# jianzhnie/ScaleRL

Hardware: NVIDIA H100
Metric: learner_frames_per_sec (higher is better)
Workload: dtype bf16

## Files before the change

### scalerl_b200/csrc/igemm_tma.cuh

```cuda
#pragma once
#include <cuda.h>
#include "common.cuh"
#include "kernels.h"

namespace srl {

SRL_DEVINL void tma_prefetch_desc(const CUtensorMap* m) {
  asm volatile("prefetch.tensormap [%0];" ::"l"(reinterpret_cast<uint64_t>(m)) : "memory");
}
SRL_DEVINL void tma_load_2d(void* dst, const CUtensorMap* m, uint64_t* bar, int c0, int c1) {
  asm volatile("cp.async.bulk.tensor.2d.shared::cluster.global.mbarrier::complete_tx::bytes [%0], [%1, {%3, %4}], [%2];"
               ::"r"(smem_u32(dst)), "l"(reinterpret_cast<uint64_t>(m)), "r"(smem_u32(bar)), "r"(c0), "r"(c1) : "memory");
}
SRL_DEVINL void tma_load_3d(void* dst, const CUtensorMap* m, uint64_t* bar, int c0, int c1, int c2) {
  asm volatile("cp.async.bulk.tensor.3d.shared::cluster.global.mbarrier::complete_tx::bytes [%0], [%1, {%3, %4, %5}], [%2];"
               ::"r"(smem_u32(dst)), "l"(reinterpret_cast<uint64_t>(m)), "r"(smem_u32(bar)), "r"(c0), "r"(c1), "r"(c2) : "memory");
}
SRL_DEVINL void tma_load_4d(void* dst, const CUtensorMap* m, uint64_t* bar, int c0, int c1, int c2, int c3) {
  asm volatile("cp.async.bulk.tensor.4d.shared::cluster.global.mbarrier::complete_tx::bytes [%0], [%1, {%3, %4, %5, %6}], [%2];"
               ::"r"(smem_u32(dst)), "l"(reinterpret_cast<uint64_t>(m)), "r"(smem_u32(bar)), "r"(c0), "r"(c1), "r"(c2), "r"(c3)
               : "memory");
}
SRL_DEVINL void tma_load_5d(void* dst, const CUtensorMap* m, uint64_t* bar, int c0, int c1, int c2, int c3, int c4) {
  asm volatile("cp.async.bulk.tensor.5d.shared::cluster.global.mbarrier::complete_tx::bytes [%0], [%1, {%3, %4, %5, %6, %7}], [%2];"
               ::"r"(smem_u32(dst)), "l"(reinterpret_cast<uint64_t>(m)), "r"(smem_u32(bar)), "r"(c0), "r"(c1), "r"(c2), "r"(c3), "r"(c4)
               : "memory");
}

constexpr int IGT_THREADS = 288;

template <class P, int SPLIT = 0>
struct TmaCfg {
  static constexpr int KROWS = P::A_MN ? P::KROWS : 64;
  static constexpr int A_BYTES = P::A_MN ? 2 * KROWS * 128 : 128 * 128;
  static constexpr int B_BLOCKS = (P::BN + 63) / 64;
  static constexpr int B_BYTES = P::B_MN ? B_BLOCKS * KROWS * 128 : P::BN * 128;
  static constexpr int HALF_BYTES = A_BYTES + B_BYTES;
  static constexpr int STAGE_BYTES = HALF_BYTES * (1 + SPLIT);
  static constexpr int NB = P::BN / 2;
  static constexpr int STAGES = fit_stages(P::STAGES, 2 * WG_IMG_BYTES + 1024 + 256, STAGE_BYTES);
  static constexpr int SMEM_BYTES = STAGES * STAGE_BYTES + 2 * WG_IMG_BYTES + 1024 + 256;
  static_assert(SMEM_BYTES <= 232448, "shared memory budget (227 KB)");
  static_assert(NB == 32 || NB == 64 || NB == 128, "MMA N per warpgroup");
  static constexpr int MMAS = P::A_MN ? KROWS / 16 : 4;
  static_assert(A_BYTES % 1024 == 0 && B_BYTES % 1024 == 0, "operand tiles must keep 1024 B alignment (SWIZZLE_128B atoms)");
  static_assert(P::A_MN == P::B_MN, "mixed majors are not used");
  static_assert(KROWS % 16 == 0, "contraction rows per stage must be a multiple of MMA K = 16");
};

template <class P, int SPLIT>
SRL_DEVINL void igt_epilogue(const typename P::Params& p, int tm, int ty, int row, int c0, float (&v)[16]) {
  if constexpr (SPLIT) P::template epilogue16<1>(p, tm, ty, row, c0, v); else P::epilogue16(p, tm, ty, row, c0, v);
}
template <class P, int SPLIT>
SRL_DEVINL void igt_epilogue(const typename P::Params& p, int tm, int ty, int row, int c0, float (&v)[16], const uint4 (&pre)[2]) {
  if constexpr (SPLIT) P::template epilogue16<1>(p, tm, ty, row, c0, v, pre); else P::epilogue16(p, tm, ty, row, c0, v, pre);
}

template <class P, int SPLIT = 0>
__global__ void __launch_bounds__(IGT_THREADS) igemm_tma_kernel(const __grid_constant__ typename P::Params p) {
  using C = TmaCfg<P, SPLIT>;
  extern __shared__ uint8_t smem_raw[];
  uint8_t* smem = reinterpret_cast<uint8_t*>((reinterpret_cast<uintptr_t>(smem_raw) + 1023) & ~uintptr_t(1023));
  float* img = reinterpret_cast<float*>(smem + C::STAGES * C::STAGE_BYTES);
  uint64_t* bars = reinterpret_cast<uint64_t*>(smem + C::STAGES * C::STAGE_BYTES + 2 * WG_IMG_BYTES);
  uint64_t* full = bars;
  uint64_t* empty = bars + C::STAGES;

  const int tid = threadIdx.x;
  const int warp = tid >> 5;
  const int tm = blockIdx.x, ty = blockIdx.y;
  const int nkb = P::num_kblocks(p, tm, ty);

  if constexpr (P::ZERO_INIT) {
    if (P::zero_cta(ty)) {
      uint4* z = reinterpret_cast<uint4*>(smem);
      for (int i = tid; i < C::STAGES * C::STAGE_BYTES / 16; i += IGT_THREADS) z[i] = make_uint4(0, 0, 0, 0);
    }
    __syncthreads();
    for (int s = 0; s < C::STAGES; ++s) P::init_smem(p, tm, ty, smem + s * C::STAGE_BYTES, tid);
    fence_proxy_async_smem();
  }
  if (warp == 8 && (tid & 31) == 0) {
    for (int s = 0; s < C::STAGES; ++s) { mbar_init(&full[s], 1); mbar_init(&empty[s], 8); }
    mbar_fence_init();
    P::prefetch(p);
  }
  __syncthreads();
  pdl_wait(P::KID);
  if (tid == 256) pdl_launch();

  if (warp == 8) {
    const uint32_t leader = elect_one_sync();
    for (int kb = 0; kb < nkb; ++kb) {
      const int s = kb % C::STAGES;
      mbar_wait(&empty[s], ((kb / C::STAGES) & 1) ^ 1);
      if (leader) {
        uint8_t* sA = smem + s * C::STAGE_BYTES;
        if constexpr (SPLIT) P::issue_split(p, tm, ty, kb, sA, C::A_BYTES, C::HALF_BYTES, &full[s]);
        else P::issue(p, tm, ty, kb, sA, sA + C::A_BYTES, &full[s]);
      }
      __syncwarp();
    }
  } else {
    const int g = warp >> 2, wt = tid & 127;
    constexpr int NB = C::NB;
    uint4 pre[P::PREFETCH ? NB / 16 : 1][2];
    if constexpr (P::PREFETCH) {
#pragma unroll
      for (int c = 0; c < NB / 16; ++c) P::prefetch16(p, tm, ty, wt, g * NB + c * 16, pre[c]);
    }
    float acc[2][NB / 2];
#pragma unroll
    for (int h = 0; h < 2; ++h)
#pragma unroll
      for (int i = 0; i < NB / 2; ++i) acc[h][i] = 0.f;
    constexpr uint32_t ASTEP = P::A_MN ? 2048 / 16 : 32 / 16, BSTEP = P::B_MN ? 2048 / 16 : 32 / 16;
    constexpr uint32_t A_HI = (P::A_MN ? C::KROWS * 128 : 64 * 128) / 16;
    const uint32_t b_off = P::B_MN ? (g * NB / 64) * C::KROWS * 128 + (g * NB % 64) * 2 : g * NB * 128;
    for (int kb = 0; kb < nkb; ++kb) {
      const int s = kb % C::STAGES;
      mbar_wait(&full[s], (kb / C::STAGES) & 1);
      const uint32_t a0 = smem_u32(smem + s * C::STAGE_BYTES);
      const uint64_t ad0 = P::A_MN ? make_smem_desc(a0, C::KROWS * 128, 1024) : make_smem_desc(a0, 16, 1024);
      const uint64_t bd0 = P::B_MN ? make_smem_desc(a0 + C::A_BYTES + b_off, C::KROWS * 128, 1024) : make_smem_desc(a0 + C::A_BYTES + b_off, 16, 1024);
      wg_fence();
#pragma unroll
      for (int k = 0; k < C::MMAS; ++k) {
        const uint64_t ad = ad0 + (uint64_t)(k * ASTEP), bd = bd0 + (uint64_t)(k * BSTEP);
        wg_mma128<NB, P::A_MN ? 1 : 0, P::B_MN ? 1 : 0>(acc, ad, A_HI, bd, (kb | k) != 0);
        if constexpr (SPLIT) {
          wg_mma128<NB, P::A_MN ? 1 : 0, P::B_MN ? 1 : 0>(acc, ad, A_HI, bd + (uint64_t)(C::HALF_BYTES / 16), 1);
          wg_mma128<NB, P::A_MN ? 1 : 0, P::B_MN ? 1 : 0>(acc, ad + (uint64_t)(C::HALF_BYTES / 16), A_HI, bd, 1);
        }
      }
      wg_commit();
      if constexpr (C::STAGES > 1) {
        wg_wait_prev();
        __syncwarp();
        if (kb > 0 && (tid & 31) == 0) mbar_arrive(&empty[(kb - 1) % C::STAGES]);
      } else {
        wg_wait_all();
        __syncwarp();
        if ((tid & 31) == 0) mbar_arrive(&empty[s]);
      }
    }
    wg_wait_all();
    wg_fence_regs(acc[0]); wg_fence_regs(acc[1]);
    float* my_img = img + g * (WG_IMG_BYTES / 4);
#pragma unroll
    for (int c = 0; c < NB / 16; ++c) {
      float v[16];
      wg_acc_row16<NB>(acc, c, my_img, wt, 2 + g, v);
      if constexpr (P::PREFETCH) igt_epilogue<P, SPLIT>(p, tm, ty, wt, g * NB + c * 16, v, pre[c]);
      else igt_epilogue<P, SPLIT>(p, tm, ty, wt, g * NB + c * 16, v);
    }
  }
}

template <class P, int SPLIT = 0>
cudaError_t igemm_tma_launch(const typename P::Params& p, dim3 grid, cudaStream_t stream) {
  using C = TmaCfg<P, SPLIT>;
  if (grid.x == 0 || grid.y == 0) return cudaSuccess;
  static PerDeviceOnce once;
  { cudaError_t e = ensure_max_dynamic_smem(once, igemm_tma_kernel<P, SPLIT>, C::SMEM_BYTES); if (e != cudaSuccess) return e; }
  return launch_chain(igemm_tma_kernel<P, SPLIT>, grid, dim3(IGT_THREADS), C::SMEM_BYTES, stream, p);
}

}
```

### scalerl_b200/csrc/tma_problems.cuh

```cuda
#pragma once
#include "igemm_tma.cuh"
#include "encoder_problems.cuh"

namespace srl {

#define SRL_TMAP alignas(64) CUtensorMap

struct TFcFwd {
  static constexpr int KID = 31;
  static constexpr bool PREFETCH = false;
  static constexpr int BN = 64, STAGES = 4, SPLITS = 4;
  static constexpr bool A_MN = false, B_MN = false, ZERO_INIT = false;
  static constexpr int KROWS = 64;
  struct Params { SRL_TMAP a3m; SRL_TMAP w; SRL_TMAP a3m_lo; SRL_TMAP w_lo; float* out; int M; };
  SRL_DEVINL static void prefetch(const Params& p) { tma_prefetch_desc(&p.a3m); tma_prefetch_desc(&p.w); }
  SRL_DEVINL static int kb_begin(int split) { return (49 * split) / SPLITS; }
  SRL_DEVINL static void issue_split(const Params& p, int tm, int ty, int kb, uint8_t* st, int a_bytes, int half, uint64_t* bar) {
    const int k = (kb_begin(ty % SPLITS) + kb) * 64;
    mbar_arrive_expect_tx(bar, 2 * (128 * 128 + 64 * 128));
    tma_load_2d(st, &p.a3m, bar, k, tm * 128);
    tma_load_2d(st + a_bytes, &p.w, bar, k, (ty / SPLITS) * 64);
    tma_load_2d(st + half, &p.a3m_lo, bar, k, tm * 128);
    tma_load_2d(st + half + a_bytes, &p.w_lo, bar, k, (ty / SPLITS) * 64);
  }
  template <int SPLIT>
  SRL_DEVINL static void epilogue16(const Params& p, int tm, int ty, int row, int c0, float (&v)[16]) { epilogue16(p, tm, ty, row, c0, v); }
  SRL_DEVINL static int num_kblocks(const Params&, int, int ty) { const int sp = ty % SPLITS; return kb_begin(sp + 1) - kb_begin(sp); }
  SRL_DEVINL static void issue(const Params& p, int tm, int ty, int kb, uint8_t* sA, uint8_t* sB, uint64_t* bar) {
    const int k = (kb_begin(ty % SPLITS) + kb) * 64;
    mbar_arrive_expect_tx(bar, 128 * 128 + 64 * 128);
    tma_load_2d(sA, &p.a3m, bar, k, tm * 128);
    tma_load_2d(sB, &p.w, bar, k, (ty / SPLITS) * 64);
  }
  SRL_DEVINL static void epilogue16(const Params& p, int tm, int ty, int row, int c0, float (&v)[16]) {
    const int m = tm * 128 + row;
    if (m >= p.M) return;
    float4* o = reinterpret_cast<float4*>(p.out + ((size_t)(ty % SPLITS) * p.M + m) * 512 + (ty / SPLITS) * 64 + c0);
#pragma unroll
    for (int j = 0; j < 4; ++j) o[j] = make_float4(v[4 * j], v[4 * j + 1], v[4 * j + 2], v[4 * j + 3]);
  }
};

struct TFcDgrad {
  static constexpr int KID = 32;
  static constexpr bool PREFETCH = true;
  static constexpr int BN = 64, STAGES = 4;
  static constexpr bool A_MN = false, B_MN = false, ZERO_INIT = false;
  static constexpr int KROWS = 64;
  struct Params { SRL_TMAP dhm; SRL_TMAP w; SRL_TMAP dhm_lo; SRL_TMAP w_lo; const bf16* a3; bf16* da3; bf16* da3_lo; int M; };
  SRL_DEVINL static void prefetch(const Params& p) { tma_prefetch_desc(&p.dhm); tma_prefetch_desc(&p.w); }
  SRL_DEVINL static int num_kblocks(const Params&, int, int) { return 8; }
  SRL_DEVINL static void issue_split(const Params& p, int tm, int ty, int kb, uint8_t* st, int a_bytes, int half, uint64_t* bar) {
    mbar_arrive_expect_tx(bar, 2 * (128 * 128 + 64 * 128));
    tma_load_2d(st, &p.dhm, bar, kb * 64, tm * 128);
    tma_load_2d(st + a_bytes, &p.w, bar, kb * 64, ty * 64);
    tma_load_2d(st + half, &p.dhm_lo, bar, kb * 64, tm * 128);
    tma_load_2d(st + half + a_bytes, &p.w_lo, bar, kb * 64, ty * 64);
  }
  SRL_DEVINL static void issue(const Params& p, int tm, int ty, int kb, uint8_t* sA, uint8_t* sB, uint64_t* bar) {
    mbar_arrive_expect_tx(bar, 128 * 128 + 64 * 128);
    tma_load_2d(sA, &p.dhm, bar, kb * 64, tm * 128);
    tma_load_2d(sB, &p.w, bar, kb * 64, ty * 64);
  }
  SRL_DEVINL static void prefetch16(const Params& p, int tm, int ty, int row, int c0, uint4 (&mk)[2]) {
    const int m = tm * 128 + row;
    if (m < p.M) ld_mask16(p.a3 + (size_t)m * 3136 + ty * 64 + c0, mk);
  }
  SRL_DEVINL static void epilogue16(const Params& p, int tm, int ty, int row, int c0, float (&v)[16], const uint4 (&mk)[2]) {
    epilogue16<0>(p, tm, ty, row, c0, v, mk);
  }
  template <int SPLIT>
  SRL_DEVINL static void epilogue16(const Params& p, int tm, int ty, int row, int c0, float (&v)[16], const uint4 (&mk)[2]) {
    const int m = tm * 128 + row;
    if (m >= p.M) return;
    relu_mask16_pre(mk, v);
    const size_t o = ((size_t)m * 81 + (ty / 7) * 9 + ty % 7) * 64 + c0;
    store_bf16x16(p.da3 + o, v);
    if constexpr (SPLIT) {
      float r[16];
#pragma unroll
      for (int j = 0; j < 16; ++j) r[j] = v[j] - __bfloat162float(__float2bfloat16_rn(v[j]));
      store_bf16x16(p.da3_lo + o, r);
    }
  }
};

SRL_DEVINL void fill_ones(uint8_t* dst, int bytes, int tid) {
  uint4* q = reinterpret_cast<uint4*>(dst);
  for (int i = tid; i < bytes / 16; i += IGT_THREADS) q[i] = make_uint4(0x3F803F80u, 0x3F803F80u, 0x3F803F80u, 0x3F803F80u);
}

struct TFcWgrad {
  static constexpr int KID = 33;
  static constexpr bool PREFETCH = false;
  static constexpr int BN = 64, STAGES = 4, KROWS = 64;
  static constexpr bool A_MN = true, B_MN = true, ZERO_INIT = true;
  struct Params { SRL_TMAP dhm; SRL_TMAP a3m; SRL_TMAP dhm_lo; SRL_TMAP a3m_lo; float* dw; float* db; int M; };
  SRL_DEVINL static void prefetch(const Params& p) { tma_prefetch_desc(&p.dhm); tma_prefetch_desc(&p.a3m); }
  SRL_DEVINL static void issue_split(const Params& p, int, int ty, int kb, uint8_t* st, int a_bytes, int half, uint64_t* bar) {
    const int hw = ty >> 2, j0 = (ty & 3) * 128;
    mbar_arrive_expect_tx(bar, (hw < 49 ? 6 : 4) * 64 * 128);
    tma_load_2d(st, &p.dhm, bar, j0, kb * 64);
    tma_load_2d(st + KROWS * 128, &p.dhm, bar, j0 + 64, kb * 64);
    tma_load_2d(st + half, &p.dhm_lo, bar, j0, kb * 64);
    tma_load_2d(st + half + KROWS * 128, &p.dhm_lo, bar, j0 + 64, kb * 64);
    if (hw < 49) {
      tma_load_2d(st + a_bytes, &p.a3m, bar, hw * 64, kb * 64);
      tma_load_2d(st + half + a_bytes, &p.a3m_lo, bar, hw * 64, kb * 64);
    }
  }
  template <int SPLIT>
  SRL_DEVINL static void epilogue16(const Params& p, int tm, int ty, int row, int c0, float (&v)[16]) { epilogue16(p, tm, ty, row, c0, v); }
  SRL_DEVINL static bool zero_cta(int) { return true; }
  SRL_DEVINL static int num_kblocks(const Params& p, int, int) { return (p.M + 63) >> 6; }
  SRL_DEVINL static void init_smem(const Params&, int, int ty, uint8_t* stage, int tid) {
    if ((ty >> 2) == 49) fill_ones(stage + 2 * KROWS * 128, KROWS * 128, tid);
  }
  SRL_DEVINL static void issue(const Params& p, int, int ty, int kb, uint8_t* sA, uint8_t* sB, uint64_t* bar) {
    const int hw = ty >> 2, j0 = (ty & 3) * 128;
    mbar_arrive_expect_tx(bar, (hw < 49 ? 3 : 2) * 64 * 128);
    tma_load_2d(sA, &p.dhm, bar, j0, kb * 64);
    tma_load_2d(sA + KROWS * 128, &p.dhm, bar, j0 + 64, kb * 64);
    if (hw < 49) tma_load_2d(sB, &p.a3m, bar, hw * 64, kb * 64);
  }
  SRL_DEVINL static void epilogue16(const Params& p, int, int ty, int row, int c0, float (&v)[16]) {
    const int j = (ty & 3) * 128 + row, hw = ty >> 2;
    if (hw < 49) {
#pragma unroll
      for (int jj = 0; jj < 16; ++jj) p.dw[(size_t)j * 3136 + (c0 + jj) * 49 + hw] = v[jj];
    } else if (c0 == 0) {
      p.db[j] = v[0];
    }
  }
};

struct TFcWgradN {
  static constexpr int KID = 36;
  static constexpr bool PREFETCH = false;
  static constexpr int BN = 256, STAGES = 4, KROWS = 64, NCT = 13;
  static constexpr bool A_MN = true, B_MN = true, ZERO_INIT = true;
  struct Params { SRL_TMAP dhm; SRL_TMAP a3tm; float* dw; float* db; int M; };
  SRL_DEVINL static void prefetch(const Params& p) { tma_prefetch_desc(&p.dhm); tma_prefetch_desc(&p.a3tm); }
  SRL_DEVINL static bool zero_cta(int ty) { return (ty >> 2) == NCT; }
  SRL_DEVINL static int num_kblocks(const Params& p, int, int) { return (p.M + 63) >> 6; }
  SRL_DEVINL static void init_smem(const Params&, int, int ty, uint8_t* stage, int tid) {
    if ((ty >> 2) == NCT) fill_ones(stage + 2 * KROWS * 128, KROWS * 128, tid);
  }
  SRL_DEVINL static void issue(const Params& p, int, int ty, int kb, uint8_t* sA, uint8_t* sB, uint64_t* bar) {
    const int ct = ty >> 2, j0 = (ty & 3) * 128;
    const int nb = ct < NCT ? (ct == NCT - 1 ? 1 : 4) : 0;
    mbar_arrive_expect_tx(bar, (2 + nb) * 64 * 128);
    tma_load_2d(sA, &p.dhm, bar, j0, kb * 64);
    tma_load_2d(sA + KROWS * 128, &p.dhm, bar, j0 + 64, kb * 64);
    for (int q = 0; q < nb; ++q) tma_load_2d(sB + q * KROWS * 128, &p.a3tm, bar, ct * 256 + q * 64, kb * 64);
  }
  SRL_DEVINL static void epilogue16(const Params& p, int, int ty, int row, int c0, float (&v)[16]) {
    const int j = (ty & 3) * 128 + row, ct = ty >> 2, col = ct * 256 + c0;
    if (ct < NCT) {
      if (col < 3136) {
        float4* d = reinterpret_cast<float4*>(p.dw + (size_t)j * 3136 + col);
#pragma unroll
        for (int q = 0; q < 4; ++q) d[q] = make_float4(v[4 * q], v[4 * q + 1], v[4 * q + 2], v[4 * q + 3]);
      }
    } else if (c0 == 0) {
      p.db[j] = v[0];
    }
  }
};

}
```

Before: 2.479 million.

## Stage fp32 accumulator tile in smem for coalesced FC weight-grad stores

Adds an optional TILE_F32 epilogue path. Both warpgroups write their fp32 accumulators into a padded shared-memory tile that reuses the pipeline stage buffers. Each warp then stores whole rows as coalesced float4 writes, instead of going through the per-row 16-column image path. The FC weight-grad problem is retiled from BN=256 to BN=128 with more column tiles and 5 stages, which doubles the grid and shrinks per-CTA registers. The cost is extra barriers and smaller N per MMA, in exchange for better occupancy and store coalescing.

```diff
diff --git a/scalerl_b200/csrc/igemm_tma.cuh b/scalerl_b200/csrc/igemm_tma.cuh
--- a/scalerl_b200/csrc/igemm_tma.cuh
+++ b/scalerl_b200/csrc/igemm_tma.cuh
@@ -1,5 +1,6 @@
 #pragma once
 #include <cuda.h>
+#include <type_traits>
 #include "common.cuh"
 #include "kernels.h"
 
@@ -28,6 +29,22 @@
 }
 
 constexpr int IGT_THREADS = 288;
+
+template <class P, class = void> struct TileF32 : std::false_type {};
+template <class P> struct TileF32<P, std::void_t<decltype(P::TILE_F32)>> : std::bool_constant<P::TILE_F32> {};
+constexpr int TILE_F32_PITCH = 136;
+
+template <int N>
+SRL_DEVINL void wg_acc_stage_f32(const float (&d)[2][N / 2], float* buf, int wt) {
+  const int w = wt >> 5, l = wt & 31;
+#pragma unroll
+  for (int h = 0; h < 2; ++h)
+#pragma unroll
+    for (int i = 0; i < N / 2; i += 2) {
+      const int row = 64 * h + 16 * w + (l >> 2) + 8 * ((i >> 1) & 1), col = 8 * (i >> 2) + 2 * (l & 3);
+      *reinterpret_cast<float2*>(buf + row * TILE_F32_PITCH + col) = make_float2(d[h][i], d[h][i + 1]);
+    }
+}
 
 template <class P, int SPLIT = 0>
 struct TmaCfg {
@@ -38,8 +55,11 @@
   static constexpr int HALF_BYTES = A_BYTES + B_BYTES;
   static constexpr int STAGE_BYTES = HALF_BYTES * (1 + SPLIT);
   static constexpr int NB = P::BN / 2;
-  static constexpr int STAGES = fit_stages(P::STAGES, 2 * WG_IMG_BYTES + 1024 + 256, STAGE_BYTES);
-  static constexpr int SMEM_BYTES = STAGES * STAGE_BYTES + 2 * WG_IMG_BYTES + 1024 + 256;
+  static constexpr bool TILE_F32 = TileF32<P>::value;
+  static constexpr int IMG_BYTES = TILE_F32 ? 0 : 2 * WG_IMG_BYTES;
+  static constexpr int STAGES = fit_stages(P::STAGES, IMG_BYTES + 1024 + 256, STAGE_BYTES);
+  static constexpr int SMEM_BYTES = STAGES * STAGE_BYTES + IMG_BYTES + 1024 + 256;
+  static_assert(!TILE_F32 || (P::BN == 128 && !SPLIT && 128 * TILE_F32_PITCH * 4 <= STAGES * STAGE_BYTES), "staged fp32 tile");
   static_assert(SMEM_BYTES <= 232448, "shared memory budget (227 KB)");
   static_assert(NB == 32 || NB == 64 || NB == 128, "MMA N per warpgroup");
   static constexpr int MMAS = P::A_MN ? KROWS / 16 : 4;
@@ -63,7 +83,7 @@
   extern __shared__ uint8_t smem_raw[];
   uint8_t* smem = reinterpret_cast<uint8_t*>((reinterpret_cast<uintptr_t>(smem_raw) + 1023) & ~uintptr_t(1023));
   float* img = reinterpret_cast<float*>(smem + C::STAGES * C::STAGE_BYTES);
-  uint64_t* bars = reinterpret_cast<uint64_t*>(smem + C::STAGES * C::STAGE_BYTES + 2 * WG_IMG_BYTES);
+  uint64_t* bars = reinterpret_cast<uint64_t*>(smem + C::STAGES * C::STAGE_BYTES + C::IMG_BYTES);
   uint64_t* full = bars;
   uint64_t* empty = bars + C::STAGES;
 
@@ -147,13 +167,24 @@
     }
     wg_wait_all();
     wg_fence_regs(acc[0]); wg_fence_regs(acc[1]);
-    float* my_img = img + g * (WG_IMG_BYTES / 4);
-#pragma unroll
-    for (int c = 0; c < NB / 16; ++c) {
-      float v[16];
-      wg_acc_row16<NB>(acc, c, my_img, wt, 2 + g, v);
-      if constexpr (P::PREFETCH) igt_epilogue<P, SPLIT>(p, tm, ty, wt, g * NB + c * 16, v, pre[c]);
-      else igt_epilogue<P, SPLIT>(p, tm, ty, wt, g * NB + c * 16, v);
+    if constexpr (C::TILE_F32) {
+      float* tile = reinterpret_cast<float*>(smem);
+      named_bar(1, 256);
+      wg_acc_stage_f32<NB>(acc, tile + g * NB, wt);
+      named_bar(1, 256);
+      const int l = tid & 31;
+#pragma unroll 4
+      for (int r = warp; r < 128; r += 8)
+        P::epilogue_row4(p, ty, r, 4 * l, *reinterpret_cast<const float4*>(tile + r * TILE_F32_PITCH + 4 * l));
+    } else {
+      float* my_img = img + g * (WG_IMG_BYTES / 4);
+#pragma unroll
+      for (int c = 0; c < NB / 16; ++c) {
+        float v[16];
+        wg_acc_row16<NB>(acc, c, my_img, wt, 2 + g, v);
+        if constexpr (P::PREFETCH) igt_epilogue<P, SPLIT>(p, tm, ty, wt, g * NB + c * 16, v, pre[c]);
+        else igt_epilogue<P, SPLIT>(p, tm, ty, wt, g * NB + c * 16, v);
+      }
     }
   }
 }
diff --git a/scalerl_b200/csrc/tma_problems.cuh b/scalerl_b200/csrc/tma_problems.cuh
--- a/scalerl_b200/csrc/tma_problems.cuh
+++ b/scalerl_b200/csrc/tma_problems.cuh
@@ -136,8 +136,8 @@
 
 struct TFcWgradN {
   static constexpr int KID = 36;
-  static constexpr bool PREFETCH = false;
-  static constexpr int BN = 256, STAGES = 4, KROWS = 64, NCT = 13;
+  static constexpr bool PREFETCH = false, TILE_F32 = true;
+  static constexpr int BN = 128, STAGES = 5, KROWS = 64, NCT = 25;
   static constexpr bool A_MN = true, B_MN = true, ZERO_INIT = true;
   struct Params { SRL_TMAP dhm; SRL_TMAP a3tm; float* dw; float* db; int M; };
   SRL_DEVINL static void prefetch(const Params& p) { tma_prefetch_desc(&p.dhm); tma_prefetch_desc(&p.a3tm); }
@@ -148,22 +148,18 @@
   }
   SRL_DEVINL static void issue(const Params& p, int, int ty, int kb, uint8_t* sA, uint8_t* sB, uint64_t* bar) {
     const int ct = ty >> 2, j0 = (ty & 3) * 128;
-    const int nb = ct < NCT ? (ct == NCT - 1 ? 1 : 4) : 0;
+    const int nb = ct < NCT ? (ct == NCT - 1 ? 1 : 2) : 0;
     mbar_arrive_expect_tx(bar, (2 + nb) * 64 * 128);
     tma_load_2d(sA, &p.dhm, bar, j0, kb * 64);
     tma_load_2d(sA + KROWS * 128, &p.dhm, bar, j0 + 64, kb * 64);
-    for (int q = 0; q < nb; ++q) tma_load_2d(sB + q * KROWS * 128, &p.a3tm, bar, ct * 256 + q * 64, kb * 64);
+    for (int q = 0; q < nb; ++q) tma_load_2d(sB + q * KROWS * 128, &p.a3tm, bar, ct * BN + q * 64, kb * 64);
   }
-  SRL_DEVINL static void epilogue16(const Params& p, int, int ty, int row, int c0, float (&v)[16]) {
-    const int j = (ty & 3) * 128 + row, ct = ty >> 2, col = ct * 256 + c0;
+  SRL_DEVINL static void epilogue_row4(const Params& p, int ty, int row, int c, float4 v) {
+    const int j = (ty & 3) * 128 + row, ct = ty >> 2, col = ct * BN + c;
     if (ct < NCT) {
-      if (col < 3136) {
-        float4* d = reinterpret_cast<float4*>(p.dw + (size_t)j * 3136 + col);
-#pragma unroll
-        for (int q = 0; q < 4; ++q) d[q] = make_float4(v[4 * q], v[4 * q + 1], v[4 * q + 2], v[4 * q + 3]);
-      }
-    } else if (c0 == 0) {
-      p.db[j] = v[0];
+      if (col < 3136) *reinterpret_cast<float4*>(p.dw + (size_t)j * 3136 + col) = v;
+    } else if (c == 0) {
+      p.db[j] = v.x;
     }
   }
 };
```

Result: no change. 2.500 million, median of 6 (+0.8%).
